# mathematiguy/pypardis

Hardware: AMD Instinct MI355X
Metric: points clustered/sec (whole node), 100M 3-D pts, 1/2/4/8 GPUs; % HBM roofline (higher is better)
Workload: dtype f32 coords, f64 predicate

## Files before the change

include/pardis.h:

```cpp
#ifndef PARDIS_H
#define PARDIS_H

#include <stdint.h>

#ifdef __cplusplus
extern "C" {
#endif

#define PD_ABI_VERSION 3

enum pd_status {
    PD_OK = 0,
    PD_EINVAL = -1,
    PD_EOOM = -2,
    PD_EHIP = -3,
    PD_ERCCL = -4,
    PD_EUNSUPPORTED = -5
};

enum pd_dtype { PD_F32 = 0, PD_F64 = 1 };

enum pd_metric { PD_EUCLIDEAN = 0, PD_CITYBLOCK = 1 };

enum pd_option {
    PD_OPT_TIMING = 1,
    PD_OPT_FULL_COUNTS = 2,
    PD_OPT_SEQUENTIAL_MOMENTS = 3,
    PD_OPT_XSUB = 6,
    PD_OPT_FP32_SCREEN = 7,
    PD_OPT_SWEEP_STATS = 8,
    PD_OPT_DENSE_PRUNE = 11   ,
    PD_OPT_COUNT_ROTATE = 12  ,
    PD_OPT_CENTRE_WINDOW = 13 ,
    PD_OPT_DIR_BUDGET = 14    ,
    PD_OPT_LABEL_BUCKETS = 15 ,
    PD_OPT_DIR_PAGED = 17     ,
    PD_OPT_DENSE_SCREEN = 18  ,
    PD_OPT_SHARD_CORE_BIT = 19 ,
    PD_OPT_COUNT_REPLAY = 24  ,
    PD_OPT_VERIFY_FUSED = 28
};

enum pd_timing_slot {
    PD_T_HALO = 0, PD_T_SORT, PD_T_GATHER, PD_T_CELLS, PD_T_COUNT, PD_T_LINK, PD_T_MERGE,
    PD_T_ROOTS, PD_T_BORDER, PD_T_LABEL, PD_T_TOTAL, PD_T_RECORDS, PD_T_CELLS_N, PD_T_GRID_CELLS,
    PD_T_KEY_BITS, PD_T_CORE_RECORDS,
    PD_T_S_COUNT_CAND, PD_T_S_LINK_CAND, PD_T_S_LINK_HIT, PD_T_S_LINK_CORE, PD_T_S_LINK_SAME,
    PD_T_S_LINK_FIND_SAME, PD_T_S_LINK_UNIONS, PD_T_S_VERIFY_PAIRS,
    PD_T_GRID_GROW,
    PD_T_COUNT_KERNEL,
    PD_T_DIR_PAGED,
    PD_T_DIR_WORDS,
    PD_T_S_COUNT_BATCHES,
    PD_T_S_COUNT_STAGED,
    PD_T_HALO_FALLBACK,
    PD_T_NSLOTS
};

typedef struct pd_ctx pd_ctx;

int32_t pd_abi_version(void);
const char* pd_last_error(void);

int32_t pd_ctx_create(int32_t device, pd_ctx** out);
int32_t pd_ctx_destroy(pd_ctx* ctx);
int32_t pd_ctx_set_option(pd_ctx* ctx, int32_t option, int64_t value);
int32_t pd_ctx_timings(pd_ctx* ctx, double* out_host, int32_t n_slots);

int32_t pd_bbox(pd_ctx* ctx, const void* X, int32_t dtype, int64_t n, int32_t d,
                double* lohi_host, int64_t* nonfinite_host, void* stream);

int32_t pd_kd_moments(pd_ctx* ctx, const void* X, int32_t dtype, int64_t n, int32_t d,
                      const int32_t* labels, int32_t n_sel, const int32_t* sel_host,
                      double* moments_host, void* stream);

int32_t pd_kd_counts(pd_ctx* ctx, const void* X, int32_t dtype, int64_t n, int32_t d,
                     const int32_t* labels, int32_t n_sel, const int32_t* sel_host,
                     const int32_t* axis_host, const double* bounds_host, int64_t* counts_host,
                     void* stream);

int32_t pd_kd_split(pd_ctx* ctx, const void* X, int32_t dtype, int64_t n, int32_t d,
                    int32_t* labels, int32_t n_sel, const int32_t* sel_host,
                    const int32_t* axis_host, const double* boundary_host,
                    const int32_t* new_host, void* stream);

int32_t pd_kd_radix_hist(pd_ctx* ctx, const void* X, int32_t dtype, int64_t n, int32_t d,
                         const int32_t* labels, int32_t n_sel, const int32_t* sel_host,
                         const int32_t* axis_host, const uint64_t* prefix_host, int32_t shift,
                         int64_t* hist_host, void* stream);

int32_t pd_sort_pairs(pd_ctx* ctx, void* keys, int32_t key_bytes, uint32_t* vals, int64_t n,
                      int32_t key_bits, void* stream);

// ... 218 lines not shown
```

pypardis_amd/_native.py:

```python
from __future__ import annotations

import ctypes
import os
import threading

import numpy as np
import torch

HERE = os.path.dirname(os.path.abspath(__file__))
LIB_PATH = os.environ.get("PYPARDIS_LIB") or os.path.join(HERE, "libpardis.so")

PD_F32, PD_F64 = 0, 1
PD_EUCLIDEAN, PD_CITYBLOCK = 0, 1
PD_OPT_TIMING, PD_OPT_FULL_COUNTS, PD_OPT_SEQUENTIAL_MOMENTS = 1, 2, 3
PD_OPT_XSUB, PD_OPT_FP32_SCREEN = 6, 7
PD_OPT_SWEEP_STATS = 8
PD_OPT_DENSE_PRUNE = 11
PD_OPT_COUNT_ROTATE = 12
PD_OPT_CENTRE_WINDOW = 13
PD_OPT_DIR_BUDGET = 14
PD_OPT_LABEL_BUCKETS = 15
PD_OPT_DIR_PAGED = 17
PD_OPT_DENSE_SCREEN = 18
PD_OPT_SHARD_CORE_BIT = 19
PD_OPT_COUNT_REPLAY = 24
PD_OPT_VERIFY_FUSED = 28
PD_OPT_HALO_PASSES = 25
PD_OPT_HALO_CAP = 26
PD_OPT_KD_FUSE = 27
PD_OPT_HALO_TREE = 29
PD_OPT_KD_REPLAY = 30
PD_OPT_RETIRED = (4, 5, 9, 10, 16, 20, 21, 22, 23, 25, 26, 27, 29, 30)
TIMING_SLOTS = ["halo", "sort", "gather", "cells", "count", "link", "merge", "roots", "border",
                "label", "total", "records", "cells_n", "grid_cells", "key_bits", "core_records",
                "s_count_cand", "s_link_cand", "s_link_hit", "s_link_core", "s_link_same",
                "s_link_find_same", "s_link_unions", "s_verify_pairs", "grid_grow",
                "count_kernel", "dir_paged", "dir_words", "s_count_batches", "s_count_staged",
                "halo_fallback"]

EXPORTS = ["pd_abi_version", "pd_last_error", "pd_ctx_create", "pd_ctx_destroy",
           "pd_ctx_set_option", "pd_ctx_timings", "pd_bbox", "pd_kd_moments", "pd_kd_counts",
           "pd_kd_split", "pd_halo_members", "pd_cluster", "pd_train", "pd_kd_moments_dd",
           "pd_route", "pd_pack", "pd_train_begin", "pd_train_exports", "pd_merge_exports",
           "pd_train_end", "pd_select_roots", "pd_sort_pairs", "pd_sort_u32", "pd_rank_labels",
           "pd_kd_radix_hist", "pd_kd_pass", "pd_owned_results", "pd_scatter_results",
           "pd_comm_unique_id", "pd_comm_init", "pd_comm_init_all", "pd_comm_destroy",
           "pd_comm_all_reduce", "pd_comm_all_gather_v", "pd_comm_all_to_all_v",
           "pd_comm_broadcast", "pd_dense_count", "pd_dense_link", "pd_dense_border",
           "pd_dense_finish", "pd_kd_build", "pd_kd_labels", "pd_train_tree", "pd_kdx_begin", "pd_kdx_moments",
           "pd_kdx_axes", "pd_kdx_counts", "pd_kdx_boundary", "pd_kdx_end", "pd_route2",
           "pd_pack2", "pd_results", "pd_results_scatter", "pd_comm_exchange", "pd_comm_abort",
           "pd_comm_self_check", "pd_comm_size", "pd_index_build", "pd_index_query",
           "pd_index_destroy", "pd_cluster_weighted", "pd_train_weighted",
           "pd_train_tree_weighted", "pd_index_kdist", "pd_index_radius_count",
           "pd_index_radius_fill", "pd_index_kneighbors", "pd_index_mreach_forest",
           "pd_forest_labels", "pd_forest_condense", "pd_condensed_select",
           "pd_condensed_labels"]


class PardisError(RuntimeError):
    def __init__(self, code, msg):
        super().__init__(f"libpardis error {code}: {msg}")
        self.code = code


_lib = None
_lock = threading.Lock()
_tls = threading.local()


def load():
    global _lib
    if _lib is not None:
        return _lib
    with _lock:
        if _lib is not None:
            return _lib
        if not os.path.exists(LIB_PATH):
            raise ImportError(
# ... 1161 lines not shown
```

pypardis_amd/csrc/api.hip:

```cpp
#include "../../include/pardis.h"

#include <cstring>
#include <string>
#include <vector>

#include "internal.hpp"

struct pd_ctx {
    pd::Ctx c;
};

namespace pd {

static thread_local std::string g_err;
void* pinned(Ctx& ctx, size_t bytes) {
    struct Hdr {
        size_t bytes;
    };
    Hdr* h = (Hdr*)ctx.pinned;
    if (!h || h->bytes < bytes) {
        if (h) {
            PD_HIP(hipDeviceSynchronize());
            PD_HIP(hipHostFree(h));
            ctx.pinned = nullptr;
// ... 90 lines not shown
}

int32_t pd_ctx_destroy(pd_ctx* ctx) {
    if (!ctx) return PD_OK;
    int32_t rc = guard(ctx, [&] {
        ctx->c.arena.release();
        if (ctx->c.pinned) (void)hipHostFree(ctx->c.pinned);
        for (auto& e : ctx->c.ev)
            if (e) (void)hipEventDestroy(e);
    });
    delete ctx;
    return rc;
}

int32_t pd_ctx_set_option(pd_ctx* ctx, int32_t option, int64_t value) {
    return guard(ctx, [&] {
        if (!ctx) throw Error(PD_EINVAL, "null context");
        if (option == PD_OPT_TIMING)
            ctx->c.timing = value != 0;
        else if (option == PD_OPT_FULL_COUNTS)
            ctx->c.full_counts = value != 0;
        else if (option == PD_OPT_SEQUENTIAL_MOMENTS)
            ctx->c.seq_moments = value != 0;
        else if (option == PD_OPT_FP32_SCREEN)
            ctx->c.screen = value != 0;
        else if (option == PD_OPT_SWEEP_STATS)
            ctx->c.sweep_stats = value != 0;
        else if (option == PD_OPT_DENSE_PRUNE) {
            if (value < 0 || value > 2) throw Error(PD_EINVAL, "dense prune is 0, 1 or 2");
            ctx->c.dense_prune = (int)value;
        } else if (option == PD_OPT_COUNT_ROTATE) {
            if (value < 0 || value > 0x7FFFFFFF) throw Error(PD_EINVAL, "count rotate must be >= 0");
            ctx->c.count_rotate = (int)value;
        } else if (option == PD_OPT_CENTRE_WINDOW) {
            if (value > 0x7FFFFFFF) throw Error(PD_EINVAL, "centre window too large");
            ctx->c.centre_window = value < 0 ? -1 : (int)value;
        } else if (option == PD_OPT_DIR_BUDGET) {
            if (value < 16) throw Error(PD_EINVAL, "directory budget must be >= 16 bytes");
            ctx->c.dir_budget = value;
        } else if (option == PD_OPT_XSUB) {
            if (value < 1 || value > 16) throw Error(PD_EINVAL, "xsub must be in [1, 16]");
            ctx->c.xsub = (int)value;
        } else if (option == PD_OPT_LABEL_BUCKETS) {
            ctx->c.label_buckets = value < 0 ? -1 : (value == 2 ? 2 : (value ? 1 : 0));
        } else if (option == PD_OPT_DIR_PAGED) {
            ctx->c.dir_paged = value < 0 ? -1 : (value ? 1 : 0);
        } else if (option == PD_OPT_DENSE_SCREEN) {
            if (value < 0 || value > 1) throw Error(PD_EINVAL, "dense screen is 0 or 1");
            ctx->c.dense_screen = (int)value;
        } else if (option == PD_OPT_SHARD_CORE_BIT) {
            ctx->c.shard_core_bit = value != 0;
        } else if (option == PD_OPT_VERIFY_FUSED) {
            ctx->c.verify_fused = value != 0;
        } else if (option == PD_OPT_COUNT_REPLAY) {
            if (value < 0 || value > 65536) throw Error(PD_EINVAL, "count replay must be in [0, 65536]");
            ctx->c.count_replay = (int)value;
        } else if (option == 4 || option == 5 || option == 9 || option == 10 || option == 16 ||
                   (option >= 20 && option <= 23) || (option >= 25 && option <= 27) || option == 29 ||
                   option == 30) {
            throw Error(PD_EINVAL, "option " + std::to_string(option) +
                                       " was retired (see pardis.h, pd_option)");
        } else
            throw Error(PD_EINVAL, "unknown option");
    });
}

int32_t pd_ctx_timings(pd_ctx* ctx, double* out, int32_t n) {
    return guard(ctx, [&] {
        if (!ctx || !out) throw Error(PD_EINVAL, "null argument");
        const Timings& t = ctx->c.t;
        const double v[PD_T_NSLOTS] = {t.halo,    t.sort,   t.gather, t.cells,
                                       t.count,   t.link,   t.merge,  t.roots,  t.border,
                                       t.label,   t.total,  (double)t.records,
                                       (double)t.cells_n, (double)t.grid_cells,
                                       (double)t.key_bits, (double)t.core_records,
                                       (double)t.sweep[0], (double)t.sweep[1],
                                       (double)t.sweep[2], (double)t.sweep[3],
                                       (double)t.sweep[4], (double)t.sweep[5],
                                       (double)t.sweep[6], (double)t.sweep[7], t.grid_grow,
                                       (double)t.count_kernel, (double)t.dir_paged,
                                       (double)t.dir_words, (double)t.sweep[8],
                                       (double)t.sweep[9], (double)t.halo_fallback};
        for (int i = 0; i < n && i < PD_T_NSLOTS; ++i) out[i] = v[i];
    });
}

int32_t pd_bbox(pd_ctx* ctx, const void* X, int32_t dtype, int64_t n, int32_t d, double* lohi,
                int64_t* bad, void* stream) {
    return guard(ctx, [&] {
        check_common(ctx, X, n, d);
        if (!lohi) throw Error(PD_EINVAL, "null lohi");
        if (n == 0) throw Error(PD_EINVAL, "bbox of an empty set");
        bbox(ctx->c, X, dtype, n, d, lohi, bad, (hipStream_t)stream);
    });
}

int32_t pd_kd_moments(pd_ctx* ctx, const void* X, int32_t dtype, int64_t n, int32_t d,
                      const int32_t* labels, int32_t n_sel, const int32_t* sel, double* out,
                      void* stream) {
    return guard(ctx, [&] {
        check_common(ctx, X, n, d);
        if (n_sel < 0 || (n_sel && (!sel || !out)) || (n && !labels))
            throw Error(PD_EINVAL, "bad selection");
        if (n == 0) {
            std::memset(out, 0, sizeof(double) * 3 * d * n_sel);
            return;
// ... 906 lines not shown
```

pypardis_amd/csrc/internal.hpp:

```cpp
#pragma once

#include "common.hpp"
#include "kdtree.hpp"

#include <map>
#include <vector>

namespace pd {

struct Arena {
    struct Buf {
        void* ptr = nullptr;
        size_t bytes = 0;
    };
    std::map<std::string, Buf> bufs;
    template <typename T>
    T* get(const std::string& name, size_t count) {
        size_t bytes = count * sizeof(T);
        if (bytes == 0) bytes = 16;
        Buf& b = bufs[name];
        if (b.bytes < bytes) {
            if (b.ptr) PD_HIP(hipFree(b.ptr));
            b.ptr = nullptr;
            size_t want = bytes + bytes / 8;
// ... 59 lines not shown
    double eps = 0;
    int rank = 0, world = 1;
    int KS = 1;
    bool mfma = false;
    double scale = 1.0;
    double* center = nullptr;
    float elo = 0, ehi = 0;
    uint32_t* cnt = nullptr;
    uint32_t n_core = 0, n_border = 0;
    uint32_t* clist = nullptr;
    uint32_t* par = nullptr;
    uint32_t* keyc = nullptr;
    uint32_t* key_out = nullptr;
    uint32_t* blist = nullptr;
    uint32_t* best = nullptr;
    const void* cf[4] = {};
    unsigned long long* tiles = nullptr;
};

struct KdxState {
    bool valid = false;
    int d = 0;
    KdLevels lv;
    std::vector<int32_t> cur;
    char* tables = nullptr;
    double* trace = nullptr;
    double* bbox = nullptr;
    double* mom = nullptr;
};

struct RouteState {
    bool valid = false;
    int64_t n = 0;
    int n_ranks = 0;
    unsigned tiles = 0;
    uint64_t* mask = nullptr;
    uint64_t* off = nullptr;
};

struct Ctx {
    int device = 0;
    Arena arena;
    void* pinned = nullptr;
    bool timing = false;
    bool full_counts = false;
    bool seq_moments = false;
    int xsub = 2;
    int centre_window = -1;
    int count_rotate = 1024;
    int count_replay = 0;
    uint64_t* rs_look = nullptr;
    uint64_t rs_look_tiles = 0;
    uint32_t rs_epoch = 0;
    bool verify_fused = false;
    bool screen = true;
    bool sweep_stats = false;
    int64_t dir_budget = 32ll << 30;
    int dir_paged = -1;
    int dense_prune = 1;
    bool shard_core_bit = false;
    int dense_screen = 1;
    int label_buckets = -1;
    Timings t;
    PhaseState st;
    DenseState dn;
    KdxState kdx;
    RouteState rt;
    hipEvent_t ev[16] = {};
};

struct TrainArgs {
    const void* X = nullptr;
    int dtype = 0;
    int64_t n = 0;
    int d = 0;
    double eps = 0;
    int min_samples = 1;
    int metric = 0;
    int P = 1;
    const double* ebox = nullptr;
    const double* data_box = nullptr;
    const int32_t* owner = nullptr;
    int32_t* labels = nullptr;
    uint8_t* core = nullptr;
    uint32_t* counts = nullptr;
    const double* weight = nullptr;
    int64_t n_clusters = 0;
    hipStream_t stream = nullptr;
    int phase = 0;
    const uint32_t* gid = nullptr;
    const uint8_t* xr = nullptr;
    const uint32_t* map_ids = nullptr;
    const uint32_t* map_keys = nullptr;
    int64_t n_map = 0;
    uint32_t* keys_out = nullptr;
    int tree_levels = 0;
    const int32_t* tree_sizes = nullptr;
    const int32_t* tree_cur = nullptr;
    const int32_t* tree_axis = nullptr;
    const double* tree_bound = nullptr;
    const int32_t* tree_new = nullptr;
    int64_t n_exports = 0;
    bool dir_paged = false;
};

void train(Ctx& ctx, TrainArgs& a);
// ... 157 lines not shown
```

pypardis_amd/csrc/kd.hip:

```cpp
#include <cstring>
#include <rocprim/rocprim.hpp>

#include <cmath>
#include <cstring>
#include <vector>

#include "internal.hpp"
#include "stream.hpp"

namespace pd {
namespace {

constexpr int kRedBlocks = 1024;
constexpr int kGroup = 4;

template <typename T, int D>
__device__ __forceinline__ void load_pt(const T* __restrict__ X, uint64_t i, uint32_t ld,
                                        double (&v)[D]) {
#pragma unroll
    for (int j = 0; j < D; ++j) v[j] = (double)X[i * ld + j];
}

__device__ __forceinline__ double wave_sum(double x) {
#pragma unroll
// ... 151 lines not shown
        }
    }
    __syncthreads();
    if (threadIdx.x < kGroup * (1 + 2 * D)) {
        const int g = threadIdx.x / (1 + 2 * D), qd = threadIdx.x % (1 + 2 * D);
        if (qd == 0) {
            double acc = 0;
            for (int k = 0; k < kBlock / 64; ++k) acc += sm[k][g * G];
            part[(uint64_t)blockIdx.x * W + g * G] = acc;
        } else {
            const int off = g * G + 1 + 2 * (qd - 1);
            DD acc{0.0, 0.0};
            for (int k = 0; k < kBlock / 64; ++k) acc = dd_add(acc, DD{sm[k][off], sm[k][off + 1]});
            part[(uint64_t)blockIdx.x * W + off] = acc.hi;
            part[(uint64_t)blockIdx.x * W + off + 1] = acc.lo;
        }
    }
}

template <typename T, int D>
__global__ void moments_seq_kernel(const T* __restrict__ X, uint64_t n, uint32_t ld,
                                   const int32_t* __restrict__ labels, int4 sel,
                                   double* __restrict__ out) {
    const int lane = threadIdx.x;
    if (lane >= kGroup * 2 * D) return;
    const int g = lane / (2 * D), rem = lane % (2 * D), j = rem % D, sq = rem / D;
    const int want = (&sel.x)[g];
    double acc = 0.0, cnt = 0.0;
    for (uint64_t i = 0; i < n; ++i) {
        if (labels[i] != want) continue;
        const T v = X[i * ld + j];
        const T vv = v * v;
        acc = acc + (sq ? (double)vv : (double)v);
        cnt += 1.0;
    }
    constexpr int G = 1 + 4 * D;
    out[g * G + 1 + 2 * D * sq + 2 * j] = acc;
    out[g * G + 2 + 2 * D * sq + 2 * j] = 0.0;
    if (rem == 0) out[g * G] = cnt;
}

struct SplitTab {
    const int32_t* slot_of;
    int ntab;
    const int32_t* axis;
    const double* boundary;
    const int32_t* newlab;
    int nsplit;
};

constexpr int kTabLds = 256;
constexpr int kDirectMax = 1;

template <typename T, int D, bool LAB, bool SP, int NG, bool BB>
__global__ __launch_bounds__(kBlock) void kd_pass_kernel(const T* __restrict__ X, uint64_t n,
                                                         int32_t* __restrict__ labels, SplitTab sp,
                                                         int4 sel, double* __restrict__ part) {
    constexpr int K = (sizeof(T) * D <= 16) ? 2 : 1;
    constexpr int TP = 4 * K * kBlock;
    constexpr int NW = kBlock / 64;
    constexpr int NGa = NG > 0 ? NG : 1;
    static_assert(NW == 4 && (NG == 0 || NG == 1 || NG == 2 || NG == 4), "wave/slot mapping");
    __shared__ T s_val[(NG > kDirectMax) ? TP * D : 1];
    __shared__ int s_wcnt[NW][NGa];
    __shared__ int s_slot[SP ? kTabLds : 1], s_ax[SP ? kTabLds : 1], s_nl[SP ? kTabLds : 1];
    __shared__ double s_bd[SP ? kTabLds : 1];
    const int tid = threadIdx.x, w = tid >> 6, lane = tid & 63;
    if constexpr (SP) {
        for (int k = tid; k < sp.ntab; k += kBlock) s_slot[k] = sp.slot_of[k];
        for (int k = tid; k < sp.nsplit; k += kBlock) {
            s_ax[k] = sp.axis[k];
            s_bd[k] = sp.boundary[k];
            s_nl[k] = sp.newlab[k];
        }
        __syncthreads();
    }
    const int sl[4] = {sel.x, sel.y, sel.z, sel.w};
    const int wslot = w % NGa, sub = w / NGa, nsub = NW / NGa;
    double cnt = 0;
    DD s[D], q2[D];
#pragma unroll
    for (int j = 0; j < D; ++j) s[j] = q2[j] = DD{0.0, 0.0};
    constexpr bool kDirect = NG >= 1 && NG <= kDirectMax;
    constexpr int ND = kDirect ? NG : 1;
    double dc[ND];
    DD ds[ND][D], dq[ND][D];
#pragma unroll
    for (int g = 0; g < ND; ++g) {
        dc[g] = 0;
#pragma unroll
        for (int j = 0; j < D; ++j) ds[g][j] = dq[g][j] = DD{0.0, 0.0};
    }
    double lo[D], hi[D], bad = 0;
#pragma unroll
    for (int j = 0; j < D; ++j) {
        lo[j] = INFINITY;
        hi[j] = -INFINITY;
    }
    const uint64_t nch = (n + 3) / 4;
    const uint64_t ntile = (n + TP - 1) / TP;
    const unsigned long long lt = (1ull << lane) - 1ull;
    for (uint64_t t = blockIdx.x; t < ntile; t += gridDim.x) {
        T v[K][4][D];
        int slot[K][4];
#pragma unroll
        for (int k = 0; k < K; ++k) {
            const uint64_t ch = t * (TP / 4) + (uint64_t)k * kBlock + tid;
            int m = 0;
            if (ch < nch) {
                m = load_chunk<T, D, true>(X, n, ch, v[k]);
            } else {
#pragma unroll
                for (int q = 0; q < 4; ++q)
#pragma unroll
                    for (int j = 0; j < D; ++j) v[k][q][j] = T(0);
            }
            int lab[4] = {0, 0, 0, 0};
            if constexpr (LAB) {
                if (m) load_labels4<true>(labels, ch, m, lab);
            }
            if constexpr (SP) {
                bool changed = false;
#pragma unroll
                for (int q = 0; q < 4; ++q) {
                    const int L = lab[q];
                    if (q >= m || L < 0 || L >= sp.ntab) continue;
                    const int a = s_slot[L];
                    if (a < 0) continue;
                    const double x = (double)pick_axis<T, D>(v[k][q], s_ax[a]);
                    if (x >= s_bd[a]) {
                        lab[q] = s_nl[a];
                        changed = true;
                    }
                }
                if (changed || !LAB) store_labels4<true>(labels, ch, m, lab);
            }
#pragma unroll
            for (int q = 0; q < 4; ++q) {
                int g = -1;
#pragma unroll
                for (int h = NGa - 1; h >= 0; --h) g = (NG > 0 && lab[q] == sl[h]) ? h : g;
                slot[k][q] = q < m ? g : -1;
            }
            if constexpr (BB) {
#pragma unroll
                for (int q = 0; q < 4; ++q) {
                    if (q >= m) continue;
#pragma unroll
                    for (int j = 0; j < D; ++j) {
                        const double x = (double)v[k][q][j];
                        if (!isfinite(x)) bad += 1;
                        lo[j] = fmin(lo[j], x);
                        hi[j] = fmax(hi[j], x);
                    }
                }
            }
        }
        if constexpr (NG >= 1 && NG <= kDirectMax) {
#pragma unroll
            for (int k = 0; k < K; ++k)
#pragma unroll
                for (int q = 0; q < 4; ++q) {
#pragma unroll
                    for (int g = 0; g < NG; ++g) {
                        const bool on = slot[k][q] == g;
                        if (NG == 1 && !on) continue;
                        dc[g] += on ? 1.0 : 0.0;
#pragma unroll
                        for (int j = 0; j < D; ++j) {
                            const T x = on ? v[k][q][j] : T(0);
                            const T xx = x * x;
                            dd_acc(ds[g][j], (double)x);
                            dd_acc(dq[g][j], (double)xx);
                        }
                    }
                }
        } else if constexpr (NG > 0) {
            int wc[NGa];
#pragma unroll
            for (int g = 0; g < NGa; ++g) wc[g] = 0;
#pragma unroll
            for (int k = 0; k < K; ++k)
#pragma unroll
                for (int q = 0; q < 4; ++q)
#pragma unroll
                    for (int g = 0; g < NGa; ++g) wc[g] += __popcll(__ballot(slot[k][q] == g));
            if (lane == 0)
#pragma unroll
                for (int g = 0; g < NGa; ++g) s_wcnt[w][g] = wc[g];
            __syncthreads();
            int run[NGa], seg[NGa];
            int acc = 0;
#pragma unroll
            for (int g = 0; g < NGa; ++g) {
                seg[g] = acc;
                int before = 0;
#pragma unroll
                for (int u = 0; u < NW; ++u) {
                    before += u < w ? s_wcnt[u][g] : 0;
                    acc += s_wcnt[u][g];
                }
                run[g] = seg[g] + before;
            }
            const int total = s_wcnt[0][wslot] + s_wcnt[1][wslot] + s_wcnt[2][wslot] +
                              s_wcnt[3][wslot];
            const int start = seg[wslot];
#pragma unroll
            for (int k = 0; k < K; ++k)
#pragma unroll
                for (int q = 0; q < 4; ++q) {
#pragma unroll
                    for (int g = 0; g < NGa; ++g) {
                        const unsigned long long b = __ballot(slot[k][q] == g);
                        if (slot[k][q] == g) {
                            const int pos = run[g] + __popcll(b & lt);
#pragma unroll
                            for (int j = 0; j < D; ++j) s_val[pos * D + j] = v[k][q][j];
                        }
                        run[g] += __popcll(b);
                    }
                }
            __syncthreads();
            for (int i = sub * 64 + lane; i < total; i += nsub * 64) {
                const T* p = s_val + (size_t)(start + i) * D;
                cnt += 1.0;
#pragma unroll
                for (int j = 0; j < D; ++j) {
                    const T x = p[j];
                    const T xx = x * x;
                    dd_acc(s[j], (double)x);
                    dd_acc(q2[j], (double)xx);
                }
            }
            __syncthreads();
        }
    }
    constexpr int G = 1 + 4 * D;
    constexpr int WM = NG * G;
    constexpr int WB = BB ? 2 * D + 1 : 0;
    constexpr int W = WM + WB;
    if constexpr (kDirect) {
        __shared__ double sd[NW][NG][G];
#pragma unroll
        for (int g = 0; g < NG; ++g) {
            const double x = wave_sum(dc[g]);
            if (lane == 0) sd[w][g][0] = x;
#pragma unroll
            for (int j = 0; j < D; ++j) {
                const DD a = wave_dd(ds[g][j]);
                const DD b = wave_dd(dq[g][j]);
                if (lane == 0) {
                    sd[w][g][1 + 2 * j] = a.hi;
                    sd[w][g][2 + 2 * j] = a.lo;
                    sd[w][g][1 + 2 * D + 2 * j] = b.hi;
                    sd[w][g][2 + 2 * D + 2 * j] = b.lo;
                }
            }
        }
        __syncthreads();
        if (w < NG) {
            const int g = w;
            if (lane == 0) {
                for (int u = 0; u < NW; ++u) {
                    cnt += sd[u][g][0];
#pragma unroll
                    for (int j = 0; j < D; ++j) {
                        s[j] = dd_add(s[j], DD{sd[u][g][1 + 2 * j], sd[u][g][2 + 2 * j]});
                        q2[j] = dd_add(q2[j], DD{sd[u][g][1 + 2 * D + 2 * j], sd[u][g][2 + 2 * D + 2 * j]});
                    }
                }
            }
        }
    }
    __shared__ double sm[NW][G + WB];
    if constexpr (NG > 0) {
        const double x = wave_sum(cnt);
        if (lane == 0) sm[w][0] = x;
#pragma unroll
        for (int j = 0; j < D; ++j) {
            const DD a = wave_dd(s[j]);
            const DD b = wave_dd(q2[j]);
            if (lane == 0) {
                sm[w][1 + 2 * j] = a.hi;
                sm[w][2 + 2 * j] = a.lo;
                sm[w][1 + 2 * D + 2 * j] = b.hi;
                sm[w][2 + 2 * D + 2 * j] = b.lo;
            }
        }
    }
    if constexpr (BB) {
#pragma unroll
        for (int j = 0; j < D; ++j) {
            const double a = wave_min(lo[j]), b = wave_max(hi[j]);
            if (lane == 0) {
                sm[w][G + j] = a;
                sm[w][G + D + j] = b;
            }
        }
        const double bb = wave_sum(bad);
        if (lane == 0) sm[w][G + 2 * D] = bb;
    }
    if constexpr (W > 0) {
        __syncthreads();
        double* out = part + (uint64_t)blockIdx.x * W;
        for (int k = tid; k < W; k += kBlock) {
            if (k < WM) {
                const int g = k / G, r = k % G;
                if (r == 0) {
                    double a = 0;
                    for (int u = g; u < NW; u += NGa) a += sm[u][0];
                    out[k] = a;
                } else if ((r - 1) % 2 == 0) {
                    DD a{0.0, 0.0};
                    for (int u = g; u < NW; u += NGa) a = dd_add(a, DD{sm[u][r], sm[u][r + 1]});
                    out[k] = a.hi;
                    out[k + 1] = a.lo;
                }
            } else {
                const int b = k - WM;
                double a = sm[0][G + b];
                for (int u = 1; u < NW; ++u)
                    a = b < D ? fmin(a, sm[u][G + b])
                              : (b < 2 * D ? fmax(a, sm[u][G + b]) : a + sm[u][G + b]);
                out[k] = a;
            }
        }
    }
}

__global__ __launch_bounds__(kBlock) void kd_finish_kernel(const double* __restrict__ part, int nb,
                                                           int WM, int G, int D, int W,
                                                           double* __restrict__ out) {
    __shared__ double sh[kBlock], sl[kBlock];
    for (int k = blockIdx.x; k < W; k += gridDim.x) {
        const bool mom = k < WM;
        const int r = mom ? k % G : 0;
        if (mom && r != 0 && (r - 1) % 2 == 1) continue;
        const bool is_dd = mom && r != 0;
        const int b = mom ? -1 : k - WM;
        DD acc{0.0, 0.0};
        double x = mom || b == 2 * D ? 0.0 : (b < D ? INFINITY : -INFINITY);
        for (int i = threadIdx.x; i < nb; i += kBlock) {
            const double* p = part + (uint64_t)i * W;
            if (is_dd)
                acc = dd_add(acc, DD{p[k], p[k + 1]});
            else if (mom || b == 2 * D)
                x += p[k];
            else
                x = b < D ? fmin(x, p[k]) : fmax(x, p[k]);
        }
        sh[threadIdx.x] = is_dd ? acc.hi : x;
        sl[threadIdx.x] = acc.lo;
// ... 387 lines not shown
                        sqq = dd_add(sqq, DD{p[1 + 2 * D + 2 * j], p[2 + 2 * D + 2 * j]});
                    }
                }
        });
        for (int g = 0; g < kGroup && g0 + g < n_sel; ++g) {
            double* o = out + (size_t)(g0 + g) * (dd_out ? Gd : 3 * d);
            const DD* su = &sum[(size_t)g * d];
            const DD* sqq = &sq[(size_t)g * d];
            if (dd_out) {
                o[0] = cnt[g];
                for (int j = 0; j < d; ++j) {
                    o[1 + 2 * j] = su[j].hi;
                    o[2 + 2 * j] = su[j].lo;
                    o[1 + 2 * d + 2 * j] = sqq[j].hi;
                    o[2 + 2 * d + 2 * j] = sqq[j].lo;
                }
                continue;
            }
            for (int j = 0; j < d; ++j) {
                o[j] = cnt[g];
                o[d + j] = su[j].hi + su[j].lo;
                o[2 * d + j] = sqq[j].hi + sqq[j].lo;
            }
        }
    }
}
}

namespace {
inline bool aligned16(const void* p) { return ((uintptr_t)p & 15u) == 0; }

inline bool vec_ok(int d, const void* X, const void* labels) {
    return d <= kMaxDim && aligned16(X) && (!labels || aligned16(labels));
}

inline bool tabs_ok(int n_sel, const int32_t* sel) {
    if (n_sel > kTabLds) return false;
    for (int k = 0; k < n_sel; ++k)
        if (sel[k] >= kTabLds) return false;
    return true;
}

template <typename F>
void dispatch_ng(int ng, F&& f) {
    switch (ng) {
        case 0: f(std::integral_constant<int, 0>{}); break;
        case 1: f(std::integral_constant<int, 1>{}); break;
        case 2: f(std::integral_constant<int, 2>{}); break;
        default: f(std::integral_constant<int, 4>{}); break;
    }
}

template <typename T, int D, bool LAB, bool SP, int NG, bool BB>
void run_pass(Ctx& ctx, const T* X, int64_t n, int32_t* labels, const SplitTab& sp, int4 sel,
              std::vector<double>& res, hipStream_t s) {
    constexpr int G = 1 + 4 * D, WM = NG * G, W = WM + (BB ? 2 * D + 1 : 0);
    constexpr int TP = 4 * kBlock * ((sizeof(T) * D <= 16) ? 2 : 1);
    static int resident = 0;
    if (!resident) {
        int per_cu = 0, dev = 0, cus = 0;
        PD_HIP(hipOccupancyMaxActiveBlocksPerMultiprocessor(
            &per_cu, reinterpret_cast<const void*>(&kd_pass_kernel<T, D, LAB, SP, NG, BB>), kBlock, 0));
        PD_HIP(hipGetDevice(&dev));
        PD_HIP(hipDeviceGetAttribute(&cus, hipDeviceAttributeMultiprocessorCount, dev));
        resident = std::max(1, per_cu) * std::max(1, cus);
    }
    const int nb = (int)std::min<int64_t>(resident, std::max<int64_t>(1, (n + TP - 1) / TP));
    double* part = ctx.arena.get<double>("pass_part", (size_t)nb * (W > 0 ? W : 1));
    hipLaunchKernelGGL((kd_pass_kernel<T, D, LAB, SP, NG, BB>), dim3(nb), dim3(kBlock), 0, s,
                       X, (uint64_t)n, labels, sp, sel, part);
    PD_HIP(hipGetLastError());
    res.assign(W, 0.0);
    if constexpr (W > 0) {
        double* fin = ctx.arena.get<double>("pass_fin", W);
        hipLaunchKernelGGL(kd_finish_kernel, dim3(W), dim3(kBlock), 0, s, part, nb, WM, G, D, W,
                           fin);
        PD_HIP(hipGetLastError());
        double* h = (double*)pinned(ctx, sizeof(double) * W);
        PD_HIP(hipMemcpyAsync(h, fin, sizeof(double) * W, hipMemcpyDeviceToHost, s));
        sync(s);
        std::memcpy(res.data(), h, sizeof(double) * W);
    }
}
}

void kd_pass(Ctx& ctx, const void* X, int dtype, int64_t n, int d, int32_t* labels,
             bool labels_zero, int n_split, const int32_t* ssel, const int32_t* saxis,
             const double* sbound, const int32_t* snew, int n_sel, const int32_t* sel,
             double* out_dd, double* lohi, int64_t* bad, hipStream_t s) {
    const bool lab_first = labels_zero && n_split == 0;
    if (n_sel == 0 && !lohi) {
        if (n_split) kd_split(ctx, X, dtype, n, d, labels, n_split, ssel, saxis, sbound, snew, s);
        return;
    }
    if (!vec_ok(d, X, labels) || ctx.seq_moments || !tabs_ok(n_split, ssel)) {
        if (n_split) kd_split(ctx, X, dtype, n, d, labels, n_split, ssel, saxis, sbound, snew, s);
        if (n_sel) moments_impl(ctx, X, dtype, n, d, labels, n_sel, sel, out_dd, true, s);
        if (lohi) bbox(ctx, X, dtype, n, d, lohi, bad, s);
        return;
    }
    SplitTab st{nullptr, 0, nullptr, nullptr, nullptr, 0};
    if (n_split) {
        LabelTables t = upload_tables(ctx, n_split, ssel, saxis, sbound, 1, snew, s);
        st = SplitTab{t.slot_of, t.ntab, t.axis, t.dbl, t.newlab, n_split};
    }
    const int Gd = 1 + 4 * d;
    dispatch_t(dtype, [&](auto tp) {
        using T = std::remove_pointer_t<decltype(tp)>;
        dispatch_d(d, [&](auto Dc) {
            constexpr int D = decltype(Dc)::value;
            constexpr int G = 1 + 4 * D;
            std::vector<double> res;
            const int ng0 = std::min(n_sel, kGroup);
            int4 sl = make_int4(-2, -2, -2, -2);
            for (int g = 0; g < ng0; ++g) (&sl.x)[g] = sel[g];
            auto take = [&](int g0, int ng) {
                for (int g = 0; g < ng; ++g) std::memcpy(out_dd + (size_t)(g0 + g) * Gd,
                                                         res.data() + (size_t)g * G,
                                                         sizeof(double) * G);
            };
// ... 189 lines not shown
    const double sd = isnan(va) ? va : (va >= 0.0 ? __dsqrt_rn(va) : 0.0);
    for (int i = 0; i < 7; ++i)
        bounds[(size_t)k * 7 + i] = __dadd_rn(ma, __dmul_rn(__dmul_rn((double)(i - 3), 0.3), sd));
    axis[k] = a;
    double* t = trace + (size_t)k * kTrace;
    t[0] = (double)a;
    t[1] = ma;
    t[2] = va;
}

__global__ void kdb_boundary_kernel(const unsigned long long* __restrict__ cnt, int S,
                                    const double* __restrict__ bounds,
                                    double* __restrict__ boundary, double* __restrict__ trace) {
    const int k = blockIdx.x * blockDim.x + threadIdx.x;
    if (k >= S) return;
    const unsigned long long* c = cnt + (size_t)k * 8;
    const double tot = (double)c[7];
    int bi = 0;
    double best = fabs(__dsub_rn(__dmul_rn(2.0, (double)c[0]), tot));
    for (int i = 1; i < 7; ++i) {
        const double v = fabs(__dsub_rn(__dmul_rn(2.0, (double)c[i]), tot));
        if (v < best) {
            best = v;
            bi = i;
        }
    }
    boundary[k] = bounds[(size_t)k * 7 + bi];
    double* t = trace + (size_t)k * kTrace;
    for (int i = 0; i < 8; ++i) t[3 + i] = (double)c[i];
    t[11] = (double)bi;
    t[12] = boundary[k];
}

template <typename T, int D>
__global__ __launch_bounds__(kBlock) void kd_label_kernel(const T* __restrict__ X, uint64_t n,
                                                          int32_t* __restrict__ labels, KdTree t) {
    const uint64_t nch = (n + 3) / 4;
    for (uint64_t ch = (uint64_t)blockIdx.x * kBlock + threadIdx.x; ch < nch;
         ch += (uint64_t)gridDim.x * kBlock) {
        T v[4][D];
        const int m = load_chunk<T, D, true>(X, n, ch, v);
        int lab[4];
#pragma unroll
        for (int q = 0; q < 4; ++q) lab[q] = kd_tree_label<T, D>(t, t.slot, t.ax_new, t.bound, v[q]);
        store_labels4<true>(labels, ch, m, lab);
    }
}

namespace {
template <typename T, int D, bool LAB, bool SP, int NG, bool BB>
void run_pass_dev(Ctx& ctx, const T* X, int64_t n, int32_t* labels, const SplitTab& sp, int4 sel,
                  double* fin, hipStream_t s) {
    constexpr int G = 1 + 4 * D, WM = NG * G, W = WM + (BB ? 2 * D + 1 : 0);
    constexpr int TP = 4 * kBlock * ((sizeof(T) * D <= 16) ? 2 : 1);
    static int resident = 0;
    if (!resident) {
        int per_cu = 0, dev = 0, cus = 0;
        PD_HIP(hipOccupancyMaxActiveBlocksPerMultiprocessor(
            &per_cu, reinterpret_cast<const void*>(&kd_pass_kernel<T, D, LAB, SP, NG, BB>), kBlock, 0));
        PD_HIP(hipGetDevice(&dev));
        PD_HIP(hipDeviceGetAttribute(&cus, hipDeviceAttributeMultiprocessorCount, dev));
        resident = std::max(1, per_cu) * std::max(1, cus);
    }
    const int nb = (int)std::min<int64_t>(resident, std::max<int64_t>(1, (n + TP - 1) / TP));
    double* part = ctx.arena.get<double>("pass_part", (size_t)nb * (W > 0 ? W : 1));
    hipLaunchKernelGGL((kd_pass_kernel<T, D, LAB, SP, NG, BB>), dim3(nb), dim3(kBlock), 0, s,
                       X, (uint64_t)n, labels, sp, sel, part);
    PD_HIP(hipGetLastError());
    if constexpr (W > 0) {
        hipLaunchKernelGGL(kd_finish_kernel, dim3(W), dim3(kBlock), 0, s, part, nb, WM, G, D, W,
                           fin);
        PD_HIP(hipGetLastError());
    }
}


inline SplitTab split_tab(const KdLevel& p) {
    return SplitTab{p.slot, p.ntab, p.axis, p.boundary, p.newlab, p.S};
}

template <typename T, int D>
void level_moments(Ctx& ctx, const T* X, int64_t n, int32_t* labels, bool labels_written,
                   const KdLevel& prev, const int32_t* sel, int S, double* out, hipStream_t s) {
    constexpr int G = 1 + 4 * D;
    const SplitTab sp = split_tab(prev);
    const SplitTab none{nullptr, 0, nullptr, nullptr, nullptr, 0};
    for (int g0 = 0; g0 < S; g0 += kGroup) {
        const int ng = std::min(S - g0, kGroup);
        int4 sl = make_int4(-2, -2, -2, -2);
        for (int g = 0; g < ng; ++g) (&sl.x)[g] = sel[g0 + g];
        dispatch_ng(ng, [&](auto NGc) {
            constexpr int NG = decltype(NGc)::value;
            if (g0 == 0 && !labels_written)
                run_pass_dev<T, D, false, true, NG, false>(ctx, X, n, labels, sp, sl, out, s);
            else if (g0 == 0)
                run_pass_dev<T, D, true, true, NG, false>(ctx, X, n, labels, sp, sl, out, s);
            else
                run_pass_dev<T, D, true, false, NG, false>(ctx, X, n, labels, none, sl,
                                                           out + (size_t)g0 * G, s);
        });
    }
}

template <typename T, int D>
void level_counts(const T* X, int64_t n, const int32_t* labels, bool labels_written,
                  const KdLevel& v, unsigned long long* out, hipStream_t s) {
    const unsigned nb4 = grid_for((n + 3) / 4, 2048);
    const int S = v.S;
    if (S <= 4) {
        auto go = [&](auto NSc) {
            constexpr int NS = decltype(NSc)::value;
            hipLaunchKernelGGL((counts_reg_kernel<T, D, NS>), dim3(nb4), dim3(kBlock), 0, s, X,
                               (uint64_t)n, labels_written ? labels : nullptr, v.slot, v.ntab,
                               v.axis, v.bounds, S, out);
        };
        if (S == 1)
            go(std::integral_constant<int, 1>{});
// ... 338 lines not shown
```

pypardis_amd/csrc/stream.hpp:

```cpp
#pragma once

#include <type_traits>

#include "common.hpp"

namespace pd {

template <typename T, int D, bool VEC>
__device__ __forceinline__ int load_chunk(const T* __restrict__ X, uint64_t n, uint64_t c,
                                          T (&v)[4][D]) {
    const uint64_t i0 = c * 4;
    const int m = n - i0 >= 4 ? 4 : (int)(n - i0);
    if (VEC && m == 4) {
        T t[4 * D];
        if constexpr (sizeof(T) == 4) {
            const float4* p = reinterpret_cast<const float4*>(X + i0 * D);
#pragma unroll
            for (int k = 0; k < D; ++k) {
                const float4 f = p[k];
                t[4 * k] = f.x;
                t[4 * k + 1] = f.y;
                t[4 * k + 2] = f.z;
                t[4 * k + 3] = f.w;
            }
        } else {
            const double2* p = reinterpret_cast<const double2*>(X + i0 * D);
#pragma unroll
            for (int k = 0; k < 2 * D; ++k) {
                const double2 f = p[k];
                t[2 * k] = f.x;
                t[2 * k + 1] = f.y;
            }
        }
#pragma unroll
        for (int q = 0; q < 4; ++q)
#pragma unroll
            for (int j = 0; j < D; ++j) v[q][j] = t[q * D + j];
    } else {
#pragma unroll
        for (int q = 0; q < 4; ++q)
#pragma unroll
            for (int j = 0; j < D; ++j) v[q][j] = q < m ? X[(i0 + q) * D + j] : T(0);
    }
    return m;
}

template <bool VEC>
__device__ __forceinline__ void load_labels4(const int32_t* __restrict__ L, uint64_t c, int m,
                                             int (&lab)[4]) {
    if (VEC && m == 4) {
        const int4 v = reinterpret_cast<const int4*>(L)[c];
        lab[0] = v.x;
        lab[1] = v.y;
        lab[2] = v.z;
        lab[3] = v.w;
    } else {
#pragma unroll
        for (int q = 0; q < 4; ++q) lab[q] = q < m ? L[c * 4 + q] : -1;
    }
}

template <bool VEC>
__device__ __forceinline__ void store_labels4(int32_t* __restrict__ L, uint64_t c, int m,
                                              const int (&lab)[4]) {
    if (VEC && m == 4) {
        reinterpret_cast<int4*>(L)[c] = make_int4(lab[0], lab[1], lab[2], lab[3]);
    } else {
#pragma unroll
        for (int q = 0; q < 4; ++q)
            if (q < m) L[c * 4 + q] = lab[q];
    }
}

template <typename T, int D>
__device__ __forceinline__ T pick_axis(const T (&v)[D], int ax) {
    using U = std::conditional_t<sizeof(T) == 4, uint32_t, uint64_t>;
    U r = 0;
#pragma unroll
    for (int j = 0; j < D; ++j) {
        U b;
        __builtin_memcpy(&b, &v[j], sizeof(T));
        r |= b & (U)0 - (U)(ax == j);
    }
    T out;
    __builtin_memcpy(&out, &r, sizeof(T));
    return out;
}

}
```

Baseline: 4.464 billion.

## Software-prefetch next tile in kd pass kernel and compare in native precision

```diff
diff --git a/include/pardis.h b/include/pardis.h
--- a/include/pardis.h
+++ b/include/pardis.h
@@ -38,7 +38,8 @@
     PD_OPT_DENSE_SCREEN = 18  ,
     PD_OPT_SHARD_CORE_BIT = 19 ,
     PD_OPT_COUNT_REPLAY = 24  ,
-    PD_OPT_VERIFY_FUSED = 28
+    PD_OPT_VERIFY_FUSED = 28  ,
+    PD_OPT_KD_PASS_BLOCKS = 31
 };
 
 enum pd_timing_slot {
diff --git a/pypardis_amd/_native.py b/pypardis_amd/_native.py
--- a/pypardis_amd/_native.py
+++ b/pypardis_amd/_native.py
@@ -25,6 +25,7 @@
 PD_OPT_SHARD_CORE_BIT = 19
 PD_OPT_COUNT_REPLAY = 24
 PD_OPT_VERIFY_FUSED = 28
+PD_OPT_KD_PASS_BLOCKS = 31
 PD_OPT_HALO_PASSES = 25
 PD_OPT_HALO_CAP = 26
 PD_OPT_KD_FUSE = 27
diff --git a/pypardis_amd/csrc/api.hip b/pypardis_amd/csrc/api.hip
--- a/pypardis_amd/csrc/api.hip
+++ b/pypardis_amd/csrc/api.hip
@@ -166,6 +166,9 @@
             ctx->c.shard_core_bit = value != 0;
         } else if (option == PD_OPT_VERIFY_FUSED) {
             ctx->c.verify_fused = value != 0;
+        } else if (option == PD_OPT_KD_PASS_BLOCKS) {
+            if (value < 0 || value > 0x7FFFFFFF) throw Error(PD_EINVAL, "kd pass blocks must be >= 0");
+            ctx->c.kd_pass_blocks = (int)value;
         } else if (option == PD_OPT_COUNT_REPLAY) {
             if (value < 0 || value > 65536) throw Error(PD_EINVAL, "count replay must be in [0, 65536]");
             ctx->c.count_replay = (int)value;
diff --git a/pypardis_amd/csrc/internal.hpp b/pypardis_amd/csrc/internal.hpp
--- a/pypardis_amd/csrc/internal.hpp
+++ b/pypardis_amd/csrc/internal.hpp
@@ -135,6 +135,7 @@
     uint64_t* rs_look = nullptr;
     uint64_t rs_look_tiles = 0;
     uint32_t rs_epoch = 0;
+    int kd_pass_blocks = 0;
     bool verify_fused = false;
     bool screen = true;
     bool sweep_stats = false;
diff --git a/pypardis_amd/csrc/kd.hip b/pypardis_amd/csrc/kd.hip
--- a/pypardis_amd/csrc/kd.hip
+++ b/pypardis_amd/csrc/kd.hip
@@ -227,6 +227,18 @@
 constexpr int kTabLds = 256;
 constexpr int kDirectMax = 1;
 
+#ifndef PD_KD_PREFETCH
+#define PD_KD_PREFETCH 1
+#endif
+template <typename T, bool LAB, bool BB>
+constexpr bool kPassPrefetch =
+    sizeof(T) == 4 && (((PD_KD_PREFETCH) >> (BB ? 0 : (LAB ? 1 : 2))) & 1);
+
+__device__ __forceinline__ float min_t(float a, float b) { return fminf(a, b); }
+__device__ __forceinline__ float max_t(float a, float b) { return fmaxf(a, b); }
+__device__ __forceinline__ double min_t(double a, double b) { return fmin(a, b); }
+__device__ __forceinline__ double max_t(double a, double b) { return fmax(a, b); }
+
 template <typename T, int D, bool LAB, bool SP, int NG, bool BB>
 __global__ __launch_bounds__(kBlock) void kd_pass_kernel(const T* __restrict__ X, uint64_t n,
                                                          int32_t* __restrict__ labels, SplitTab sp,
@@ -239,13 +251,13 @@
     __shared__ T s_val[(NG > kDirectMax) ? TP * D : 1];
     __shared__ int s_wcnt[NW][NGa];
     __shared__ int s_slot[SP ? kTabLds : 1], s_ax[SP ? kTabLds : 1], s_nl[SP ? kTabLds : 1];
-    __shared__ double s_bd[SP ? kTabLds : 1];
+    __shared__ T s_bd[SP ? kTabLds : 1];
     const int tid = threadIdx.x, w = tid >> 6, lane = tid & 63;
     if constexpr (SP) {
         for (int k = tid; k < sp.ntab; k += kBlock) s_slot[k] = sp.slot_of[k];
         for (int k = tid; k < sp.nsplit; k += kBlock) {
             s_ax[k] = sp.axis[k];
-            s_bd[k] = sp.boundary[k];
+            s_bd[k] = bound_up<T>(sp.boundary[k]);
             s_nl[k] = sp.newlab[k];
         }
         __syncthreads();
@@ -266,34 +278,33 @@
 #pragma unroll
         for (int j = 0; j < D; ++j) ds[g][j] = dq[g][j] = DD{0.0, 0.0};
     }
-    double lo[D], hi[D], bad = 0;
+    T lo[D], hi[D];
+    uint32_t bad = 0;
 #pragma unroll
     for (int j = 0; j < D; ++j) {
-        lo[j] = INFINITY;
-        hi[j] = -INFINITY;
+        lo[j] = T(INFINITY);
+        hi[j] = T(-INFINITY);
     }
     const uint64_t nch = (n + 3) / 4;
     const uint64_t ntile = (n + TP - 1) / TP;
     const unsigned long long lt = (1ull << lane) - 1ull;
+    constexpr bool PF = kPassPrefetch<T, LAB, BB>;
+    PassTile<T, D, K> cur, nxt;
+    if (PF && blockIdx.x < ntile) load_tile<T, D, K, LAB>(X, n, nch, labels, blockIdx.x, tid, cur);
     for (uint64_t t = blockIdx.x; t < ntile; t += gridDim.x) {
-        T v[K][4][D];
+        const uint64_t tn = t + gridDim.x;
+        if constexpr (PF) {
+            if (tn < ntile) load_tile<T, D, K, LAB>(X, n, nch, labels, tn, tid, nxt);
+        } else {
+            load_tile<T, D, K, LAB>(X, n, nch, labels, t, tid, cur);
+        }
+        T(&v)[K][4][D] = cur.v;
         int slot[K][4];
 #pragma unroll
         for (int k = 0; k < K; ++k) {
             const uint64_t ch = t * (TP / 4) + (uint64_t)k * kBlock + tid;
-            int m = 0;
-            if (ch < nch) {
-                m = load_chunk<T, D, true>(X, n, ch, v[k]);
-            } else {
-#pragma unroll
-                for (int q = 0; q < 4; ++q)
-#pragma unroll
-                    for (int j = 0; j < D; ++j) v[k][q][j] = T(0);
-            }
-            int lab[4] = {0, 0, 0, 0};
-            if constexpr (LAB) {
-                if (m) load_labels4<true>(labels, ch, m, lab);
-            }
+            const int m = cur.m[k];
+            int(&lab)[4] = cur.lab[k];
             if constexpr (SP) {
                 bool changed = false;
 #pragma unroll
@@ -302,7 +313,7 @@
                     if (q >= m || L < 0 || L >= sp.ntab) continue;
                     const int a = s_slot[L];
                     if (a < 0) continue;
-                    const double x = (double)pick_axis<T, D>(v[k][q], s_ax[a]);
+                    const T x = pick_axis<T, D>(v[k][q], s_ax[a]);
                     if (x >= s_bd[a]) {
                         lab[q] = s_nl[a];
                         changed = true;
@@ -323,10 +334,10 @@
                     if (q >= m) continue;
 #pragma unroll
                     for (int j = 0; j < D; ++j) {
-                        const double x = (double)v[k][q][j];
-                        if (!isfinite(x)) bad += 1;
-                        lo[j] = fmin(lo[j], x);
-                        hi[j] = fmax(hi[j], x);
+                        const T x = v[k][q][j];
+                        bad += isfinite(x) ? 0u : 1u;
+                        lo[j] = min_t(lo[j], x);
+                        hi[j] = max_t(hi[j], x);
                     }
                 }
             }
@@ -409,6 +420,9 @@
             }
             __syncthreads();
         }
+        if constexpr (PF) {
+            if (tn < ntile) cur = nxt;
+        }
     }
     constexpr int G = 1 + 4 * D;
     constexpr int WM = NG * G;
@@ -466,13 +480,13 @@
     if constexpr (BB) {
 #pragma unroll
         for (int j = 0; j < D; ++j) {
-            const double a = wave_min(lo[j]), b = wave_max(hi[j]);
+            const double a = wave_min((double)lo[j]), b = wave_max((double)hi[j]);
             if (lane == 0) {
                 sm[w][G + j] = a;
                 sm[w][G + D + j] = b;
             }
         }
-        const double bb = wave_sum(bad);
+        const double bb = wave_sum((double)bad);
         if (lane == 0) sm[w][G + 2 * D] = bb;
     }
     if constexpr (W > 0) {
@@ -966,9 +980,7 @@
 }
 
 template <typename T, int D, bool LAB, bool SP, int NG, bool BB>
-void run_pass(Ctx& ctx, const T* X, int64_t n, int32_t* labels, const SplitTab& sp, int4 sel,
-              std::vector<double>& res, hipStream_t s) {
-    constexpr int G = 1 + 4 * D, WM = NG * G, W = WM + (BB ? 2 * D + 1 : 0);
+int pass_blocks(const Ctx& ctx, int64_t n) {
     constexpr int TP = 4 * kBlock * ((sizeof(T) * D <= 16) ? 2 : 1);
     static int resident = 0;
     if (!resident) {
@@ -979,7 +991,15 @@
         PD_HIP(hipDeviceGetAttribute(&cus, hipDeviceAttributeMultiprocessorCount, dev));
         resident = std::max(1, per_cu) * std::max(1, cus);
     }
-    const int nb = (int)std::min<int64_t>(resident, std::max<int64_t>(1, (n + TP - 1) / TP));
+    const int cap = ctx.kd_pass_blocks > 0 ? std::min(ctx.kd_pass_blocks, resident) : resident;
+    return (int)std::min<int64_t>(cap, std::max<int64_t>(1, (n + TP - 1) / TP));
+}
+
+template <typename T, int D, bool LAB, bool SP, int NG, bool BB>
+void run_pass(Ctx& ctx, const T* X, int64_t n, int32_t* labels, const SplitTab& sp, int4 sel,
+              std::vector<double>& res, hipStream_t s) {
+    constexpr int G = 1 + 4 * D, WM = NG * G, W = WM + (BB ? 2 * D + 1 : 0);
+    const int nb = pass_blocks<T, D, LAB, SP, NG, BB>(ctx, n);
     double* part = ctx.arena.get<double>("pass_part", (size_t)nb * (W > 0 ? W : 1));
     hipLaunchKernelGGL((kd_pass_kernel<T, D, LAB, SP, NG, BB>), dim3(nb), dim3(kBlock), 0, s,
                        X, (uint64_t)n, labels, sp, sel, part);
@@ -1275,17 +1295,7 @@
 void run_pass_dev(Ctx& ctx, const T* X, int64_t n, int32_t* labels, const SplitTab& sp, int4 sel,
                   double* fin, hipStream_t s) {
     constexpr int G = 1 + 4 * D, WM = NG * G, W = WM + (BB ? 2 * D + 1 : 0);
-    constexpr int TP = 4 * kBlock * ((sizeof(T) * D <= 16) ? 2 : 1);
-    static int resident = 0;
-    if (!resident) {
-        int per_cu = 0, dev = 0, cus = 0;
-        PD_HIP(hipOccupancyMaxActiveBlocksPerMultiprocessor(
-            &per_cu, reinterpret_cast<const void*>(&kd_pass_kernel<T, D, LAB, SP, NG, BB>), kBlock, 0));
-        PD_HIP(hipGetDevice(&dev));
-        PD_HIP(hipDeviceGetAttribute(&cus, hipDeviceAttributeMultiprocessorCount, dev));
-        resident = std::max(1, per_cu) * std::max(1, cus);
-    }
-    const int nb = (int)std::min<int64_t>(resident, std::max<int64_t>(1, (n + TP - 1) / TP));
+    const int nb = pass_blocks<T, D, LAB, SP, NG, BB>(ctx, n);
     double* part = ctx.arena.get<double>("pass_part", (size_t)nb * (W > 0 ? W : 1));
     hipLaunchKernelGGL((kd_pass_kernel<T, D, LAB, SP, NG, BB>), dim3(nb), dim3(kBlock), 0, s,
                        X, (uint64_t)n, labels, sp, sel, part);
diff --git a/pypardis_amd/csrc/stream.hpp b/pypardis_amd/csrc/stream.hpp
--- a/pypardis_amd/csrc/stream.hpp
+++ b/pypardis_amd/csrc/stream.hpp
@@ -72,6 +72,48 @@
     }
 }
 
+template <typename T, int D, int K>
+struct PassTile {
+    T v[K][4][D];
+    int lab[K][4];
+    int m[K];
+};
+
+template <typename T, int D, int K, bool LAB>
+__device__ __forceinline__ void load_tile(const T* __restrict__ X, uint64_t n, uint64_t nch,
+                                          const int32_t* __restrict__ labels, uint64_t t, int tid,
+                                          PassTile<T, D, K>& a) {
+#pragma unroll
+    for (int k = 0; k < K; ++k) {
+        const uint64_t ch = t * (uint64_t)(K * kBlock) + (uint64_t)k * kBlock + tid;
+        a.m[k] = 0;
+        if (ch < nch) {
+            a.m[k] = load_chunk<T, D, true>(X, n, ch, a.v[k]);
+        } else {
+#pragma unroll
+            for (int q = 0; q < 4; ++q)
+#pragma unroll
+                for (int j = 0; j < D; ++j) a.v[k][q][j] = T(0);
+        }
+#pragma unroll
+        for (int q = 0; q < 4; ++q) a.lab[k][q] = 0;
+        if constexpr (LAB) {
+            if (a.m[k]) load_labels4<true>(labels, ch, a.m[k], a.lab[k]);
+        }
+    }
+}
+
+template <typename T>
+__device__ __forceinline__ T bound_up(double b) {
+    if constexpr (sizeof(T) == 8) {
+        return b;
+    } else {
+        float f = (float)b;
+        if ((double)f < b) f = nextafterf(f, INFINITY);
+        return f;
+    }
+}
+
 template <typename T, int D>
 __device__ __forceinline__ T pick_axis(const T (&v)[D], int ax) {
     using U = std::conditional_t<sizeof(T) == 4, uint32_t, uint64_t>;
```

Result: no change. 4.436 billion, median of 2 (-0.6%).
